# jonathan-laurent/AlphaZero.jl

Measured on AMD Instinct MI355X. Metric: self-play MCTS sims/sec (Connect-Four, 4096 parallel games per GPU), higher is better.
Workload: dtype f32

## Files before the change

### alphazero.jl_amd/csrc/azhip.hip

```cpp
#include "engine.h"

static thread_local std::string g_err;
int fail(int code, const char* fmt, ...) {
  char buf[512];
  va_list ap;
  va_start(ap, fmt);
  vsnprintf(buf, sizeof buf, fmt, ap);
  va_end(ap);
  g_err = buf;
  return code;
}
extern "C" const char* az_last_error(void) { return g_err.c_str(); }
extern "C" int az_abi_version(void) { return AZ_ABI_VERSION; }
extern "C" int az_abi_struct_size(int32_t which) {
  switch (which) {
    case AZ_STRUCT_ENGINE_CFG: return (int)sizeof(az_engine_cfg);
    case AZ_STRUCT_MOVE_REC: return (int)sizeof(az_move_rec);
    case AZ_STRUCT_GAME_REC: return (int)sizeof(az_game_rec);
    case AZ_STRUCT_TRACE_BUF: return (int)sizeof(az_trace_buf);
    case AZ_STRUCT_SELFPLAY_STATS: return (int)sizeof(az_selfplay_stats);
    case AZ_STRUCT_SAMPLE: return (int)sizeof(az_sample);
    case AZ_STRUCT_DATASET_INFO: return (int)sizeof(az_dataset_info);
    case AZ_STRUCT_LEARNING_STATUS: return (int)sizeof(az_learning_status_t);
    case AZ_STRUCT_TRAIN_CFG: return (int)sizeof(az_train_cfg);
// ... 349 lines not shown
    AZCHK(dalloc(e, &e->d_next, (size_t)2 * e->io_cap)); AZCHK(dalloc(e, &e->d_term, e->io_cap)); AZCHK(dalloc(e, &e->d_reward, e->io_cap));
    AZCHK(dalloc(e, &e->d_nodebuf, 512));
    AZCHK(dalloc(e, &e->d_visits, (size_t)e->io_cap * (AZ_MAX_ACTIONS + 1)));
    e->nn_cap = e->io_cap;
    AZCHK(dalloc(e, &e->d_hfeat, (size_t)e->nn_cap * gi.P * std::max(64, c->num_filters), false));
    AZCHK(dalloc(e, &e->d_X, (size_t)e->nn_cap * gi.C * gi.P)); AZCHK(dalloc(e, &e->d_A, (size_t)e->nn_cap * gi.A));
    AZCHK(dalloc(e, &e->d_P, (size_t)e->nn_cap * std::max(16, gi.APAD))); AZCHK(dalloc(e, &e->d_V, e->nn_cap)); AZCHK(dalloc(e, &e->d_Pinv, e->nn_cap));
    AZCHK(dalloc(e, &e->d_tmp_env, e->nn_cap)); AZCHK(dalloc(e, &e->d_iota, e->nn_cap)); AZCHK(dalloc(e, &e->d_ntmp, 1));
    HIPCHK(hipHostMalloc((void**)&e->h_env, sizeof(GEnv) * (size_t)e->nn_cap, hipHostMallocDefault));
    HIPCHK(hipHostMalloc((void**)&e->h_n, sizeof(int), hipHostMallocDefault));
    HIPCHK(hipHostMalloc((void**)&e->h_pv, sizeof(float) * (size_t)e->nn_cap * (gi.A + 1), hipHostMallocDefault));
    hipLaunchKernelGGL(k_iota, dim3((e->nn_cap + 255) / 256), dim3(256), 0, e->stream, e->d_iota, e->nn_cap);
    memset(&e->net, 0, sizeof e->net);
    memset(&e->net16, 0, sizeof e->net16);
    { const char* tw = getenv("AZHIP_TOWER"); e->tower_pick = tw ? atoi(tw) : 0; }
    { const char* mx = getenv("AZHIP_TOWER_MIXED"); e->tower_mixed = mx && atoi(mx) != 0; }
    { const char* hd = getenv("AZHIP_HEADS"); e->heads_pick = hd ? atoi(hd) : 0; }
    { const char* ep = getenv("AZHIP_XCH_EPOCH0"); e->xch_epoch = ep ? strtoull(ep, nullptr, 0) : 0; }
    { hipDeviceProp_t pr; HIPCHK(hipGetDeviceProperties(&pr, c->device)); e->num_cu = pr.multiProcessorCount; }
    AZCHK(net_set_kernel_attrs(e));
    { const char* ta = getenv("AZHIP_TREE_ATOMIC"); const int m = ta ? atoi(ta) : 0; v.bk_mode = m == 1 || m == 2 ? m : 0; }
    { const char* ts = getenv("AZHIP_TREE_SORT"); e->tree_sort = ts && atoi(ts) != 0 ? 1 : 0; }
    if (e->tree_sort) { AZCHK(dalloc(e, &e->d_perm, (size_t)2 * G)); AZCHK(dalloc(e, &e->d_perm_prev, (size_t)2 * G)); }
    int ng = c->batch_size > 0 ? G / c->batch_size : 1;
    if (ng < 1) ng = 1;
    if (ng > AZ_MAX_GROUPS) ng = AZ_MAX_GROUPS;
    while (ng > 1 && G % ng != 0) --ng;
    const int Gh = G / ng;
    const int blk_group = (Gh * gi.APAD + 255) / 256, blk_all = (G * gi.APAD + 255) / 256;
    e->stat_words = (size_t)4 * ((size_t)blk_group * ng + blk_all);
    AZCHK(dalloc(e, &v.stat, e->stat_words));
// ... 498 lines not shown
  }
  if (e->fr_on) {
    FRArgs fa;
    fa.st = e->d_fr; fa.done = e->d_done; fa.done_off = e->d_done_off;
    fa.recs = e->d_phase ? e->d_phase : e->d_stage; fa.recs_cap = e->d_phase ? (long long)e->phase_cap : (long long)e->v.G * e->v.max_moves;
    fa.done_cap = e->done_cap; fa.total_games = e->total_games; fa.first_game_id = (uint32_t)e->first_game_id; fa.group = g; fa.host_words = e->d_fr_words;
    static const int bg_prio = getenv("AZHIP_BG_PRIO") ? atoi(getenv("AZHIP_BG_PRIO")) : 0;
    hipStream_t s3 = side ? e->fr_s[2] : s2;
    if (side) { HIPCHK(hipStreamWaitEvent(s2, e->fr_ev[0], 0)); HIPCHK(hipStreamWaitEvent(s3, e->fr_ev[0], 0)); }
    { DView mv = v; mv.low_prio = bg_prio ? 0 : 1; LAUNCH_ON(e, s3, AZ_K_MOVE, G, (k_move_fr<Gm>), (G + 255) / 256, 256, 0, mv, e->p, fa); }
    if (e->fr_kbg > 0) {
      AZCHK(ec_next_launch(e, &e->gv[g]));
      DView bv = e->gv[g];
      bv.run_k = e->fr_kbg; bv.low_prio = bg_prio ? 0 : 1;
      if (side && e->bg_signal) { bv.bg_stop = e->d_bg_stop; bv.bg_seq = e->bg_seq; }
      LAUNCH_ON(e, s2, AZ_K_EXPAND, G, (k_tree<Gm>), gb, 256, 0, bv, e->p, 0, 1, par ^ 1);
    }
    if (side) {
      HIPCHK(hipEventRecord(e->fr_ev[1], s2)); HIPCHK(hipStreamWaitEvent(st, e->fr_ev[1], 0));
      HIPCHK(hipEventRecord(e->fr_ev[2], s3)); HIPCHK(hipStreamWaitEvent(st, e->fr_ev[2], 0));
    }
    else if (split && e->cfg.oracle == AZ_ORACLE_RESNET) HIPCHK(hipStreamWaitEvent(st, e->ev_net[g], 0));
  }
  return AZ_OK;
}
template <class Gm> static int recover_split(az_engine* e) {
  AZCHK(sync_all(e));
  *e->h_xflag = 0;
  int xerr[AZ_MAX_GROUPS + 1], skipped[2 * (AZ_MAX_GROUPS + 1)];
  HIPCHK(hipMemcpy(xerr, e->d_xerr, sizeof xerr, hipMemcpyDeviceToHost));
  HIPCHK(hipMemcpy(skipped, e->d_skipped, sizeof skipped, hipMemcpyDeviceToHost));
// ... 503 lines not shown
    fs.next_game = e->next_game;
    HIPCHK(hipMemsetAsync(e->v.finished, 0, sizeof(int) * G, e->stream));
    AZCHK(start_games<Gm>(e, aslots_refill, agids, nullptr, 1, 1));
    dirty = true;
  }
  if (!e->d_phase && (done > 0 || nrec > 0)) {
    fs.resv = 0; e->fr_prev_done = 0; e->fr_prev_recs = 0; dirty = true;
  }
  if (dirty) {
    HIPCHK(hipMemcpyAsync(e->d_fr, &fs, sizeof fs, hipMemcpyHostToDevice, e->stream));
    HIPCHK(hipStreamSynchronize(e->stream));
  }
  e->active_slots = 0;
  for (int g = 0; g < AZ_MAX_GROUPS; ++g) { e->group_active[g] = g < e->ngroups ? std::max(0, fs.active[g]) : 0; e->active_slots += e->group_active[g]; }
  e->h_fr_words[0] = e->fr_prev_done; e->h_fr_words[1] = e->active_slots;
  return vm_grow(e, e->fr_round_waves * e->fr_k + 2);
}
template <class Gm> static int fr_step(az_engine* e, int nwaves) {
  for (int w = 0; w < nwaves; ++w) {
    if (e->active_slots == 0) break;
    const int seen_done = ((volatile int*)e->h_fr_words)[0], seen_active = ((volatile int*)e->h_fr_words)[1];
    if (seen_active == 0 || (e->total_games > 0 && e->d_phase && seen_done + e->fr_given_up >= e->total_games)) break;
    AZCHK(wave<Gm>(e, e->ngroups, 0));
    if (++e->fr_since_round >= e->fr_round_waves) AZCHK(fr_round<Gm>(e));
  }
  return fr_round<Gm>(e);
}

extern "C" int az_selfplay_step(az_engine* e, int32_t nwaves) {
  ENGINE(e);
  if (!e->running) return fail(AZ_ERR_STATE, "az_selfplay_begin has not been called");
// ... 371 lines not shown
```

### alphazero.jl_amd/csrc/engine.h

```cpp
#pragma once
#include <hip/hip_runtime.h>

#include <algorithm>
#include <chrono>
#include <cmath>
#include <cstdarg>
#include <cstdio>
#include <cstring>
#include <new>
#include <string>
#include <map>
#include <mutex>
#include <vector>
#include <unordered_set>

#include "../../include/az_numerics.h"
#include "../../include/azhip.h"
#include "games.h"
#include "resnet.h"
#include "resnet16.h"
#include "resnet16b.h"
#include "tree.h"

int fail(int code, const char* fmt, ...);
// ... 27 lines not shown
  }
  return false;
}

enum TowerForm : int {
  TW_AUTO = 0,
  TW_SPLIT = 2,
  TW_NTS = 3,
  TW_NTM = 7,
  TW_11 = 16,
  TW_P19 = 19,
  TW_P21C = 20,
  TW_P21 = 21,
  TW_B22 = 22,
  TW_32 = 32,
  TW_MIXED = -1
};
struct ProfRec { hipEvent_t a = nullptr, b = nullptr; int cls = 0; };
struct az_engine {
  az_engine_cfg cfg;
  GameInfo gi;
  int device;
  hipStream_t stream;
  DView v;
  DParams p;
  int ngroups;
  DView gv[AZ_MAX_GROUPS];
  hipStream_t gs[AZ_MAX_GROUPS];
  hipStream_t gt[AZ_MAX_GROUPS];
  hipEvent_t ev_tree[AZ_MAX_GROUPS], ev_net[AZ_MAX_GROUPS];
  float* g_hfeat[AZ_MAX_GROUPS];
// ... 14 lines not shown
  int tree_sort; int* d_perm; long long* d_perm_prev;
  ECEnt* d_ec; uint32_t ec_mask; uint32_t ec_seq; int* d_ec_claim; float* d_Phit; float* d_Vhit;
  size_t stat_words; std::vector<long long> h_stat;
  std::vector<int32_t> aborted_ids;
  std::vector<void*> net_allocs;
  bool net_loaded;
  std::vector<float> blob;
  NetDev net;
  Net16bDev net16b;
  Net16Dev net16;
  uint16_t* d_geo[GEO_COUNT];
  long long tower_hist[4];
  char last_tower[96];
  int heads_pick;
  int tower_pick;
  bool tower_mixed;
  int num_cu;
  int nn_cap;
  float* d_hfeat; float* d_X; float* d_A; float* d_P; float* d_V; float* d_Pinv;
  GEnv* d_tmp_env; int* d_iota; int* d_ntmp;
  GEnv* h_env; int* h_n; float* h_pv;
  int* d_slots; uint32_t* d_gids; GEnv* d_roots; uint32_t* d_moves; double* d_eta; int* d_offsets;
  az_move_rec* d_stage; unsigned long long* d_keys; int* d_actions; unsigned long long* d_next; signed char* d_term; float* d_reward;
  char* d_nodebuf;
  int* d_visits;
  int io_cap;
  bool running;
  int total_games, next_game, first_game_id, games_done, wave_in_move, active_slots;
  std::map<int, hipGraphExec_t> wave_graphs; int use_graphs;
  bool pending[AZ_MAX_GROUPS];
  int wave_par[AZ_MAX_GROUPS];
// ... 133 lines not shown
```

### alphazero.jl_amd/csrc/net_c4.hip

```cpp
#include "net_impl.h"
AZ_NET_GAME_TU(ConnectFour, c4)


template <int F, int NT> static int tower_timeline(az_engine* e, int32_t n, unsigned long long* out, int64_t cap) {
  using T = T16<ConnectFour, F, NT>;
  const int nb = (n + T::TB - 1) / T::TB;
  if (cap < (int64_t)nb * 8) return fail(AZ_ERR_CAPACITY, "need %d words", nb * 8);
  unsigned long long* d = nullptr;
  AZCHK(dalloc(e, &d, (size_t)nb * 8));
  HIPCHK(hipMemsetAsync(d, 0, sizeof(unsigned long long) * nb * 8, e->stream));
  std::vector<GEnv> envs(n, ConnectFour::init());
  HIPCHK(hipMemcpyAsync(e->d_tmp_env, envs.data(), sizeof(GEnv) * n, hipMemcpyHostToDevice, e->stream));
  HIPCHK(hipMemcpyAsync(e->d_ntmp, &n, sizeof(int), hipMemcpyHostToDevice, e->stream));
  Net16Dev nd = e->net16;
  for (int rep = 0; rep < 2; ++rep) {
    nd.dbg = rep ? d : nullptr;
    hipLaunchKernelGGL((k_tower16<ConnectFour, F, false, NT>), dim3(nb), dim3(T::THREADS), T::BYTES, e->stream, nd, e->d_tmp_env, e->d_iota, e->d_ntmp, n, (const float*)nullptr, e->d_hfeat);
  }
  HIPCHK(hipMemcpyAsync(out, d, sizeof(unsigned long long) * nb * 8, hipMemcpyDeviceToHost, e->stream));
  HIPCHK(hipStreamSynchronize(e->stream));
  e->allocs.pop_back();
  (void)hipFree(d);
  return AZ_OK;
}
// ... 106 lines not shown
```

### alphazero.jl_amd/csrc/net_impl.h

```cpp
#pragma once
#include "engine.h"

template <class T> static constexpr double geo_frac() { return T::Geo::tab.cost / (9.0 * (T::RPAD / 16)); }
template <class T_, int ID_, bool OK_, int HIST_> struct FormFp32 {
  using T = T_;
  static constexpr int ID = ID_, HIST = HIST_;
  static constexpr bool OK = OK_, BF16 = false;
  static const Net16Dev& net(const az_engine* e) { return e->net16; }
  static constexpr double frac() { return geo_frac<T>(); }
};
template <class Gm, int F, int NT, int ID_, int HIST_> struct Form16 : FormFp32<T16<Gm, F, NT>, ID_, (NT > 0), HIST_> {
  template <bool FP> static constexpr auto K = &k_tower16<Gm, F, FP, NT>;
  static void name(char* s, size_t n, const char* g) { snprintf(s, n, "k_tower16<%s,%d,NT=%d>", g, F, NT); }
};
template <class Gm, int F> struct FormSplit : FormFp32<T16S<Gm, F>, TW_SPLIT, F == 128, 0> {
  template <bool FP> static constexpr auto K = &k_tower16s<Gm, F, FP>;
  static void name(char* s, size_t n, const char* g) { snprintf(s, n, "k_tower16s<%s,%d>", g, F); }
};
template <class Gm, int F, int NT0, int NT1, int ID_> struct FormPaired : FormFp32<T16P<Gm, F, NT0, NT1>, ID_, F == 64, 2> {
  template <bool FP> static constexpr auto K = &k_tower16x2<Gm, F, FP, NT0, NT1>;
  static void name(char* s, size_t n, const char* g) {
    if (NT0 == 11) snprintf(s, n, "k_tower16x2<%s,%d>", g, F);
    else snprintf(s, n, "k_tower16x2<%s,%d,NT=%d>", g, F, NT0 + NT1);
  }
};
template <class Gm, int F> struct FormPairedC : FormFp32<T16P<Gm, F>, TW_P21C, F == 64, 2> {
  template <bool FP> static constexpr auto K = &k_tower16x2c<Gm, F, FP>;
  static void name(char* s, size_t n, const char* g) { snprintf(s, n, "k_tower16x2c<%s,%d>", g, F); }
};
template <class Gm, int F> struct FormMixed : FormFp32<T16P<Gm, F>, TW_MIXED, F == 64, 2> {
  using T7 = T16P<Gm, F, 10, 9>;
  template <bool FP> static constexpr auto K = &k_tower16x2m<Gm, F, FP>;
  static void name(char* s, size_t n, const char* g) { snprintf(s, n, "k_tower16x2m<%s,%d>", g, F); }
};
template <class Gm, int F> struct Form32 {
  struct T { static constexpr int TB = TOWER_ROWS / Gm::P, THREADS = TowerCfg<F>::THREADS, BYTES = TowerLds<F>::BYTES; };
  static constexpr int ID = TW_32, HIST = 3;
  static constexpr bool OK = true, BF16 = false;
  template <bool FP> static constexpr auto K = &k_tower<Gm, F, FP>;
  static const NetDev& net(const az_engine* e) { return e->net; }
  static constexpr double frac() { return 1.0; }
  static void name(char* s, size_t n, const char* g) { snprintf(s, n, "k_tower<%s,%d>", g, F); }
};
template <class Gm, int F, int NT, int ID_, int HIST_> struct Form16b {
  using T = T16B<Gm, F, NT>;
  static constexpr int ID = ID_, HIST = HIST_;
  static constexpr bool OK = NT != 22 || F == 128, BF16 = true;
  template <bool FP> static constexpr auto K = &k_tower16b<Gm, F, FP, NT>;
  static const Net16bDev& net(const az_engine* e) { return e->net16b; }
// ... 2 lines not shown
};
template <class... D> struct FormList {};
template <class Gm, int F> using Forms = FormList<
    FormSplit<Gm, F>, Form16<Gm, F, NTS<Gm>, TW_NTS, 1>, Form16<Gm, F, NTM<Gm>, TW_NTM, 3>, Form16<Gm, F, 11, TW_11, 2>,
    FormPaired<Gm, F, 11, 10, TW_P21>, FormPaired<Gm, F, 10, 9, TW_P19>, FormPairedC<Gm, F>, Form32<Gm, F>,
    Form16b<Gm, F, NTS<Gm>, TW_NTS, 1>, Form16b<Gm, F, 11, TW_11, 2>, Form16b<Gm, F, 22, TW_B22, 3>>;

template <class D, bool FP> static int set_form_attr() {
  if constexpr (D::OK) HIPCHK(hipFuncSetAttribute(reinterpret_cast<const void*>(D::template K<FP>), hipFuncAttributeMaxDynamicSharedMemorySize, D::T::BYTES));
  return AZ_OK;
}
template <class Gm, int F, class... D> static int set_kernel_attrs_f(FormList<D...>) {
  int r = AZ_OK;
  (void)(((r = set_form_attr<D, false>()) == AZ_OK && (r = set_form_attr<D, true>()) == AZ_OK) && ...);
  AZCHK(r);
  AZCHK((set_form_attr<FormMixed<Gm, F>, false>()));
  HIPCHK(hipFuncSetAttribute(reinterpret_cast<const void*>(&k_heads16<Gm, F, true>), hipFuncAttributeMaxDynamicSharedMemorySize, H16<Gm, F, true>::BYTES));
  HIPCHK(hipFuncSetAttribute(reinterpret_cast<const void*>(&k_heads16<Gm, F, false>), hipFuncAttributeMaxDynamicSharedMemorySize, H16<Gm, F, false>::BYTES));
  return AZ_OK;
}
template <class T> static int upload_geo(az_engine* e) {
  using G = typename T::Geo;
  if (e->d_geo[T::GEO]) return AZ_OK;
  std::vector<uint16_t> h((size_t)10 * G::RPAD);
  for (int i = 0; i < G::RPAD; ++i) h[i] = G::tab.pos[i];
  for (int i = 0; i < 9 * G::RPAD; ++i) h[G::RPAD + i] = G::tab.nbr[i];
  uint16_t* d = nullptr;
  AZCHK(dalloc(e, &d, h.size(), false));
  HIPCHK(hipMemcpyAsync(d, h.data(), h.size() * sizeof(uint16_t), hipMemcpyHostToDevice, e->stream));
  HIPCHK(hipStreamSynchronize(e->stream));
  e->d_geo[T::GEO] = d;
// ... 89 lines not shown
template <class Gm, int F>
static int launch_heads(az_engine* e, hipStream_t st, const float* hfeat, const GEnv* envs, const int* eslots, const int* n_ptr, int n_max,
                        const float* Amask, float* Pout, float* Vout, float* Pinv, int pstride) {
  const bool small = e->heads_pick == 16 || (e->heads_pick != 32 && (n_max <= HEADS16_MAX_BOARDS || e->ngroups == 1));
  const int tiles = (n_max + 15) / 16;
  if (e->net.hd16_ok && small && 2 * tiles <= (e->num_cu > 0 ? e->num_cu : 256))
    LAUNCH_ON(e, st, AZ_K_HEADS, n_max, (k_heads16<Gm, F, true>), 2 * tiles, (H16<Gm, F, true>::THREADS), (H16<Gm, F, true>::BYTES), e->net, envs, eslots, n_ptr, n_max, Amask, hfeat, Pout, Vout, Pinv, pstride);
  else if (e->net.hd16_ok && small)
    LAUNCH_ON(e, st, AZ_K_HEADS, n_max, (k_heads16<Gm, F, false>), tiles, (H16<Gm, F, false>::THREADS), (H16<Gm, F, false>::BYTES), e->net, envs, eslots, n_ptr, n_max, Amask, hfeat, Pout, Vout, Pinv, pstride);
  else if (e->net.hd_ok)
    LAUNCH_ON(e, st, AZ_K_HEADS, n_max, (k_heads_mfma<Gm, F>), (n_max + 31) / 32, 64 * (F / 32 + HEADS_NPT<Gm>), 0, e->net, envs, eslots, n_ptr, n_max, Amask, hfeat, Pout, Vout, Pinv, pstride);
  else
    LAUNCH_ON(e, st, AZ_K_HEADS, n_max, (k_heads<Gm, F>), (n_max + 3) / 4, 4 * (F + HEADS_LP<Gm>), 0, e->net, envs, eslots, n_ptr, n_max, Amask, hfeat, Pout, Vout, Pinv, pstride);
  return AZ_OK;
}
struct TowerIn { float* hfeat; const GEnv* envs; const int* eslots; const int* n_ptr; const float* X; int* xerr; };
static const char* game_name(const az_engine* e) {
  static const char* const gn[] = {"ConnectFour", "TicTacToe", "Mancala", "Go9Planes"};
  return gn[e->cfg.game];
}
template <class D, bool FROM_PLANES> static int launch_form(az_engine* e, hipStream_t st, int n, const TowerIn& in) {
  if constexpr (!D::OK) return fail(AZ_ERR_STATE, "tower form %d does not exist for this network", (int)D::ID);
  else {
    using T = typename D::T;
    D::name(e->last_tower, sizeof e->last_tower, game_name(e));
    e->tower_hist[D::HIST]++;
    e->next_exec = D::frac();
    const int tiles = (n + T::TB - 1) / T::TB;
    if constexpr (D::ID == TW_SPLIT) {
      unsigned long long* xa; unsigned long long ep;
      AZCHK(xch_slot<typename T::Game>(e, in.hfeat, &xa, &ep));
      LAUNCH_ON(e, st, AZ_K_TOWER, n, (D::template K<FROM_PLANES>), T::SPLIT * tiles, T::THREADS, T::BYTES, D::net(e), in.envs, in.eslots, in.n_ptr, n, in.X, in.hfeat,
                xa, ep, in.xerr, e->d_xflag);
    } else
      LAUNCH_ON(e, st, AZ_K_TOWER, n, (D::template K<FROM_PLANES>), tiles, T::THREADS, T::BYTES, D::net(e), in.envs, in.eslots, in.n_ptr, n, in.X, in.hfeat);
    return AZ_OK;
  }
}
template <class Gm, int F, bool FROM_PLANES, class... D>
static int launch_tower(FormList<D...>, az_engine* e, hipStream_t st, int form, int n, const TowerIn& in) {
  const bool bf16 = e->cfg.net_bf16 != 0;
  int r = 1;
  (void)((D::ID == form && D::BF16 == bf16 && ((r = launch_form<D, FROM_PLANES>(e, st, n, in)), true)) || ...);
  return r <= 0 ? r : fail(AZ_ERR_STATE, "no tower form %d", form);
}
template <class Gm, int F, bool FROM_PLANES> static int launch_tower(az_engine* e, hipStream_t st, int form, int n, const TowerIn& in) {
  return launch_tower<Gm, F, FROM_PLANES>(Forms<Gm, F>{}, e, st, form, n, in);
}
template <class Gm, int F, bool FROM_PLANES>
static int launch_net_f(az_engine* e, hipStream_t st, float* hfeat, const GEnv* envs, const int* eslots, const int* n_ptr, int n_max, const float* X,
                        const float* Amask, float* Pout, float* Vout, float* Pinv, int pstride) {
  if (n_max <= 0) return AZ_OK;
  AZCHK((launch_tower<Gm, F, FROM_PLANES>(e, st, pick_tower<Gm, F>(e, n_max), n_max, TowerIn{hfeat, envs, eslots, n_ptr, X, e->v.err})));
  return launch_heads<Gm, F>(e, st, hfeat, envs, eslots, n_ptr, n_max, Amask, Pout, Vout, Pinv, pstride);
}
template <class Gm, bool FROM_PLANES>
static int launch_net(az_engine* e, hipStream_t st, float* hfeat, const GEnv* envs, const int* eslots, const int* n_ptr, int n_max, const float* X,
                      const float* Amask, float* Pout, float* Vout, float* Pinv, int pstride) {
  if (e->cfg.num_filters == 128) return launch_net_f<Gm, 128, FROM_PLANES>(e, st, hfeat, envs, eslots, n_ptr, n_max, X, Amask, Pout, Vout, Pinv, pstride);
  return launch_net_f<Gm, 64, FROM_PLANES>(e, st, hfeat, envs, eslots, n_ptr, n_max, X, Amask, Pout, Vout, Pinv, pstride);
}


template <class Gm, int F> static int wave_net_f(az_engine* e, int g, bool split, int nmax) {
  constexpr int L = Gm::APAD;
  const DView& v = e->gv[g];
  hipStream_t st = e->gs[g], sn = e->gt[g];
  const int G = v.G;
// ... 1 lines not shown
  const int N = std::max(1, std::min(G, nmax));
  const int* nev = v.n_eval + e->wave_par[g];
  const int* const eslots = v.eval_slots + (size_t)e->wave_par[g] * v.eval_stride;
  int npick = N;
  if (v.nleaf_host) { const int seen = ((volatile int*)e->h_nleaf)[g]; if (seen >= 0) npick = std::max(1, std::min(N, seen + seen / 8 + 8)); }
  int tw = pick_tower<Gm, F>(e, npick, N);
  if (tw == TW_P21 && e->fr_on && e->ngroups == 1 && e->tower_pick == 0 && e->fr_kbg > 0 && v.nleaf_host && v.needy_host) {
    const int cu = e->num_cu > 0 ? e->num_cu : 256;
    const int seen = ((volatile int*)e->h_nleaf)[g], needy = ((volatile int*)e->h_needy)[g];
    if (seen > 0) {
      constexpr int TB21 = T16P<Gm, 64>::TB;
      const int wgs = (seen + TB21 - 1) / TB21, rounds = (wgs + cu - 1) / cu, bg = (std::max(needy, 0) * L + 255) / 256;
      if (wgs > rounds * (cu - bg) - 14) tw = TW_P21C;
    }
  }
  const TowerIn in{e->g_hfeat[g], v.leaf_env, eslots, nev, nullptr, v.xerr};
  bool mixed = false;
  if constexpr (FormMixed<Gm, F>::OK) {
    using M = FormMixed<Gm, F>;
    using T8 = typename M::T; using T7 = typename M::T7;
    const int cu = e->num_cu > 0 ? e->num_cu : 256, first = cu * T8::TB;
    const int seen = v.nleaf_host ? ((volatile int*)e->h_nleaf)[g] : -1;
    if (tw == TW_P21 && e->tower_mixed && e->tower_pick == 0 && N > first && seen > first && seen + 16 <= first + cu * T7::TB) {
      mixed = true;
      M::name(e->last_tower, sizeof e->last_tower, game_name(e));
      e->tower_hist[M::HIST]++;
      e->next_exec = (first * geo_frac<T8>() + (seen - first) * geo_frac<T7>()) / (double)seen;
      LAUNCH_ON(e, sn, AZ_K_TOWER, N, (M::template K<false>), cu + (N - first + T7::TB - 1) / T7::TB, T8::THREADS, T8::BYTES, M::net(e), in.envs, in.eslots, in.n_ptr, N, in.X, in.hfeat, cu);
    }
  }
  if (!mixed) AZCHK((launch_tower<Gm, F, false>(e, sn, tw, N, in)));
  const bool fr = e->fr_on && split;
  if (e->bg_signal) {
    HIPCHK(hipEventRecord(e->fr_ev[3], sn));
    HIPCHK(hipStreamWaitEvent(e->fr_s[3], e->fr_ev[3], 0));
    hipLaunchKernelGGL(k_set_word, dim3(1), dim3(1), 0, e->fr_s[3], e->d_bg_stop, e->bg_seq);
  }
  if (split && !fr) { HIPCHK(hipEventRecord(e->ev_net[g], sn)); HIPCHK(hipStreamWaitEvent(st, e->ev_net[g], 0)); }
  AZCHK((launch_heads<Gm, F>(e, fr ? sn : st, e->g_hfeat[g], v.leaf_env, eslots, nev, N, (const float*)nullptr, v.Pout, v.Vout, (float*)nullptr, L)));
  if (fr) HIPCHK(hipEventRecord(e->ev_net[g], sn));
  return AZ_OK;
}
template <class Gm> static int wave_net(az_engine* e, int g, bool split, int nmax) {
  return e->cfg.num_filters == 128 ? wave_net_f<Gm, 128>(e, g, split, nmax) : wave_net_f<Gm, 64>(e, g, split, nmax);
}

// ... 16 lines not shown
```

### alphazero.jl_amd/csrc/resnet16.h

```cpp
#pragma once
#include <hip/hip_runtime.h>
#include <stdint.h>
#include "../../include/az_numerics.h"
#include "games.h"
#include "resnet.h"


enum GeoSlot {
  GEO_11,
  GEO_NTS,
  GEO_21,
  GEO_6,
  GEO_NTM,
  GEO_19,
  GEO_22,
  GEO_COUNT
};
struct Net16Dev {
  int nblocks;
  const float* stem_w;
  const float* stem_ss;
  const float4* conv_w;
  const float* conv_ss;
  const float4* head_w;
// ... 558 lines not shown

template <class T, bool FROM_PLANES>
__device__ __forceinline__ void tower16x2_body(const Net16Dev& net, const GEnv* __restrict__ leaf_env, const int* __restrict__ eval_slots, int n,
                                               const float* __restrict__ X, float* __restrict__ hfeat, int board0, const uint16_t* __restrict__ geo) {
  extern __shared__ __attribute__((aligned(16))) float lds[];
  float* buf = lds;
  float* planes = lds + T::BUF;
  uint16_t* nbr = (uint16_t*)(planes + T::PLANES);
  uint16_t* pos = nbr + 9 * T::RPAD;
  tower16_fill<T, FROM_PLANES>(buf, planes, nbr, pos, geo, leaf_env, eval_slots, X, n, board0, threadIdx.x);
  __syncthreads();
  const int wave = threadIdx.x >> 6, lane = threadIdx.x & 63;
  if (wave < T::CT) tower16_wave<T, FROM_PLANES, T::NT0, 0>(net, buf, planes, nbr, pos, wave, lane, n, board0, hfeat);
  else tower16_wave<T, FROM_PLANES, T::NT1, T::NT0>(net, buf, planes, nbr, pos, wave - T::CT, lane, n, board0, hfeat);
}
template <class Gm, int F, bool FROM_PLANES, int NT0 = 11, int NT1 = 10>
__global__ void __launch_bounds__(2 * T16Threads<F>::V, 1)
k_tower16x2(Net16Dev net, const GEnv* __restrict__ leaf_env, const int* __restrict__ eval_slots,
            const int* __restrict__ n_eval_ptr, int n_fixed, const float* __restrict__ X, float* __restrict__ hfeat) {
  using T = T16P<Gm, F, NT0, NT1>;
  const int n = FROM_PLANES ? n_fixed : *n_eval_ptr;
  const int board0 = blockIdx.x * T::TB;
  if (board0 >= n) return;
  tower16x2_body<T, FROM_PLANES>(net, leaf_env, eval_slots, n, X, hfeat, board0, net.geo[T::GEO]);
}
template <class Gm, int F, bool FROM_PLANES>
__global__ void __launch_bounds__(2 * T16Threads<F>::V, 1) __attribute__((amdgpu_num_vgpr(88)))
k_tower16x2c(Net16Dev net, const GEnv* __restrict__ leaf_env, const int* __restrict__ eval_slots,
             const int* __restrict__ n_eval_ptr, int n_fixed, const float* __restrict__ X, float* __restrict__ hfeat) {
  using T = T16P<Gm, F, 11, 10>;
  const int n = FROM_PLANES ? n_fixed : *n_eval_ptr;
  const int board0 = blockIdx.x * T::TB;
  if (board0 >= n) return;
  tower16x2_body<T, FROM_PLANES>(net, leaf_env, eval_slots, n, X, hfeat, board0, net.geo[T::GEO]);
}
template <class Gm, int F, bool FROM_PLANES>
__global__ void __launch_bounds__(2 * T16Threads<F>::V, 1)
k_tower16x2m(Net16Dev net, const GEnv* __restrict__ leaf_env, const int* __restrict__ eval_slots,
             const int* __restrict__ n_eval_ptr, int n_fixed, const float* __restrict__ X, float* __restrict__ hfeat, int first) {
  using T8 = T16P<Gm, F, 11, 10>;
  using T7 = T16P<Gm, F, 10, 9>;
  const int n = FROM_PLANES ? n_fixed : *n_eval_ptr;
  if ((int)blockIdx.x < first) {
    const int board0 = blockIdx.x * T8::TB;
    if (board0 >= n) return;
    tower16x2_body<T8, FROM_PLANES>(net, leaf_env, eval_slots, n, X, hfeat, board0, net.geo[T8::GEO]);
  } else {
    const int board0 = first * T8::TB + ((int)blockIdx.x - first) * T7::TB;
    if (board0 >= n) return;
    tower16x2_body<T7, FROM_PLANES>(net, leaf_env, eval_slots, n, X, hfeat, board0, net.geo[T7::GEO]);
  }
}

template <class Gm, int F> struct T16S : T16<Gm, F, NTS<Gm>> {
  static constexpr int SPLIT = 2, TPW = NTS<Gm>, CWL = F / 16 / SPLIT;
  static constexpr int WAVES = CWL, THREADS = 64 * WAVES;
  static constexpr int XCH_WORDS = 2 * TPW * 4 * THREADS;
};
template <class Gm, int F, bool FROM_PLANES>
__global__ void __launch_bounds__((T16S<Gm, F>::THREADS), 1)
k_tower16s(Net16Dev net, const GEnv* __restrict__ leaf_env, const int* __restrict__ eval_slots,
           const int* __restrict__ n_eval_ptr, int n_fixed, const float* __restrict__ X, float* __restrict__ hfeat,
           unsigned long long* __restrict__ xch, unsigned long long epoch, int* __restrict__ err, int* __restrict__ hflag) {
  using T = T16S<Gm, F>;
  extern __shared__ __attribute__((aligned(16))) float lds[];
  float* buf = lds;
  float* planes = lds + T::BUF;
  uint16_t* nbr = (uint16_t*)(planes + T::PLANES);
// ... 345 lines not shown
```

### alphazero.jl_amd/csrc/tree.h

```cpp
#pragma once
#include <hip/hip_runtime.h>
#include <stdint.h>
#include <type_traits>
#include "../../include/az_numerics.h"
#include "../../include/azhip.h"
#include "games.h"

enum { LEAF_NONE = 0, LEAF_NEW = 1, LEAF_TERMINAL = 2 };
enum { DERR_NODE_POOL = 1, DERR_HASH_FULL = 2, DERR_DEPTH = 3, DERR_MOVES = 4, DERR_NO_ROOT = 5 };

struct DParams {
  double gamma, cpuct, eps, alpha, prior_temp;
  int nsims, temp_len;
  int temp_xs[AZ_SCHED_MAX];
  double temp_ys[AZ_SCHED_MAX];
  uint64_t seed;
  int oracle, reset_every;
  double flip_p;
  int retire;
};

enum { SR_ACTIVE = 1, SR_MS_SHIFT = 8 };
struct alignas(64) SlotRec {
  unsigned long long root_a, root_b;
// ... 223 lines not shown
    double e = 0.0;
    if (a < Gm::A && ((m >> a) & 1)) e = eta[k++];
    v.eta[(size_t)slot * L + a] = e;
  }
}

template <class Gm> __device__ inline void set_link(char* nd, int act, uint32_t link) {
  using NL = NodeL<Gm>;
  ((uint16_t*)(nd + NL::OFF_LO))[act] = (uint16_t)(link & 0xffff);
  typename NL::hi_t* hp = (typename NL::hi_t*)(nd + NL::OFF_HI);
  *hp = (typename NL::hi_t)((*hp & ~((typename NL::hi_t)3 << (2 * act))) | ((typename NL::hi_t)(link >> 16) << (2 * act)));
}

struct KArgs { DView v; DParams p; };
template <class Gm>
__global__ void __launch_bounds__(256) __attribute__((amdgpu_num_vgpr(160))) k_tree(DView v_arg, DParams p_arg, int do_backup, int do_select, int par) {
  if (!v_arg.low_prio) __builtin_amdgcn_s_setprio(3);
  const DView& v = v_arg;
  constexpr int L = Gm::APAD;
  using NL = NodeL<Gm>;
  __shared__ int s_new[4], s_hit[4], s_evl[4], s_sims[4], s_trav[4], s_need[4], s_base, s_nbase;
  const int tid = blockIdx.x * blockDim.x + threadIdx.x;
  const int lgrp = tid / L, lane = tid % L;
  const int wl = threadIdx.x & 63, w = threadIdx.x >> 6, gbase = wl & ~(L - 1);
  int nlive = v.G;
  const int* map = v.perm;
  if (v.fr && !do_backup && v.bg_list) { nlive = v.bg_cnt[par ^ 1]; map = v.bg_list + (size_t)(par ^ 1) * v.eval_stride; }
  const bool live = lgrp < nlive;
  const int slot_in = live ? (map ? map[lgrp] : lgrp) : 0;
  const bool links_ok = v.cap_nodes <= LINK_MAX;
  unsigned long long* dbg = (v.dbg && blockIdx.x == 0 && threadIdx.x == 0) ? v.dbg : nullptr;
  if (dbg) dbg[0] = __builtin_readcyclecounter();
  if (__hip_atomic_load(v.xerr, __ATOMIC_RELAXED, __HIP_MEMORY_SCOPE_AGENT) == (int)DERR_EXCHANGE) {
    if (blockIdx.x == 0 && threadIdx.x == 0 && (do_backup || !v.fr)) atomicAdd(v.skipped + (do_select ? 0 : 1), 1);
    return;
  }

  const SlotRec s0 = v.sr[slot_in];
  unsigned long long st = (v.path + (size_t)slot_in * v.max_depth)[lane < v.max_depth ? lane : 0];
  GEnv lenv = v.leaf_env[slot_in];
  int kind = s0.leaf_kd & 3, depth = (s0.leaf_kd >> 2) & 0x0fffffff, e0 = s0.eidx, nc = s0.node_count;
  GEnv root0 = s0.root();
  uint32_t epoch0 = s0.epoch, ins = s0.leaf_ins;
  int ridx = s0.root_idx, active0 = s0.active;
  int claim0 = -1; uint32_t cmeta0 = 0;
  if (v.ec) { const int2 c2 = ((const int2*)v.ec_claim)[slot_in]; claim0 = c2.x; cmeta0 = (uint32_t)c2.y; }
#define AZ_PIN(x) asm volatile("" : "+v"(x))
  AZ_PIN(kind); AZ_PIN(depth); AZ_PIN(e0); AZ_PIN(nc); AZ_PIN(st); AZ_PIN(root0.a); AZ_PIN(root0.b); AZ_PIN(root0.fin);
// ... 283 lines not shown
  if (isnew) {
    int base = s_base;
    for (int i = 0; i < w; ++i) base += s_new[i];
    const int e = base + __popcll(bal & ((1ULL << wl) - 1ULL));
    sr->eidx = e;
    (v.eval_slots + (size_t)par * v.eval_stride)[e] = slot;
  }
  if (needy && v.fr) {
    int base = s_nbase;
    for (int i = 0; i < w; ++i) base += s_need[i];
    (v.bg_list + (size_t)par * v.eval_stride)[base + __popcll(baln & ((1ULL << wl) - 1ULL))] = slot;
  }
  if (v.ec && head && kind == LEAF_NEW) ((int2*)v.ec_claim)[slot] = make_int2(ishit ? -1 : claim, ishit ? 0 : (int)cmeta);
  if (dbg) dbg[6] = __builtin_readcyclecounter();
}

template <class Gm>
__host__ __device__ inline float rollout_value(GEnv g, uint64_t seed, uint32_t game_id, uint32_t move, uint32_t sim) {
  const bool wp = Gm::white_playing(g);
  az_rng r = az_rng_make(seed, game_id, move, AZ_RNG_ROLLOUT);
  r.ctr[3] = sim * 1024u;
  double wr = 0.0;
  for (int ply = 0; ply < 1024 && !(g.fin & 1); ++ply) {
    const uint32_t m = Gm::mask(g);
    int acts[AZ_MAX_ACTIONS], n = 0;
    for (int a = 0; a < Gm::A; ++a) if ((m >> a) & 1) acts[n++] = a;
    int k = (int)(az_rng_f64(&r) * (double)n);
    if (k >= n) k = n - 1;
    Gm::play(g, acts[k]);
    wr = (double)Gm::white_reward(g);
// ... 383 lines not shown
```

Before: 8.843 million.

## Add low-VGPR background tree kernel and adaptive paired tower split

Introduces k_tree_bg, a copy of the tree kernel capped at 56 VGPRs, for background expansion so it can co-reside with the tower kernel. In the background path, one thread reads the exchange-error flag into shared memory instead of every thread reading it. It also replaces the separate mixed tower kernel with an adaptive paired split inside k_tower16x2 that balances heavy and light tiles across CU slots, on by default when the free-running single-group mode is active. The VM growth bound is widened to account for background launches. The 56-VGPR cap may cause register spills, and the extra split logic adds per-block overhead.

Measured after the change: 8.792 million. About the same (-0.6%).

```diff
diff --git a/alphazero.jl_amd/csrc/azhip.hip b/alphazero.jl_amd/csrc/azhip.hip
--- a/alphazero.jl_amd/csrc/azhip.hip
+++ b/alphazero.jl_amd/csrc/azhip.hip
@@ -387,7 +387,7 @@
     memset(&e->net, 0, sizeof e->net);
     memset(&e->net16, 0, sizeof e->net16);
     { const char* tw = getenv("AZHIP_TOWER"); e->tower_pick = tw ? atoi(tw) : 0; }
-    { const char* mx = getenv("AZHIP_TOWER_MIXED"); e->tower_mixed = mx && atoi(mx) != 0; }
+    { const char* mx = getenv("AZHIP_TOWER_MIXED"); e->tower_mixed = mx ? (atoi(mx) != 0 ? 1 : 0) : -1; }
     { const char* hd = getenv("AZHIP_HEADS"); e->heads_pick = hd ? atoi(hd) : 0; }
     { const char* ep = getenv("AZHIP_XCH_EPOCH0"); e->xch_epoch = ep ? strtoull(ep, nullptr, 0) : 0; }
     { hipDeviceProp_t pr; HIPCHK(hipGetDeviceProperties(&pr, c->device)); e->num_cu = pr.multiProcessorCount; }
@@ -916,7 +916,7 @@
       DView bv = e->gv[g];
       bv.run_k = e->fr_kbg; bv.low_prio = bg_prio ? 0 : 1;
       if (side && e->bg_signal) { bv.bg_stop = e->d_bg_stop; bv.bg_seq = e->bg_seq; }
-      LAUNCH_ON(e, s2, AZ_K_EXPAND, G, (k_tree<Gm>), gb, 256, 0, bv, e->p, 0, 1, par ^ 1);
+      LAUNCH_ON(e, s2, AZ_K_EXPAND, G, (k_tree_bg<Gm>), gb, 256, 0, bv, e->p, 0, 1, par ^ 1);
     }
     if (side) {
       HIPCHK(hipEventRecord(e->fr_ev[1], s2)); HIPCHK(hipStreamWaitEvent(st, e->fr_ev[1], 0));
@@ -1450,7 +1450,7 @@
   e->active_slots = 0;
   for (int g = 0; g < AZ_MAX_GROUPS; ++g) { e->group_active[g] = g < e->ngroups ? std::max(0, fs.active[g]) : 0; e->active_slots += e->group_active[g]; }
   e->h_fr_words[0] = e->fr_prev_done; e->h_fr_words[1] = e->active_slots;
-  return vm_grow(e, e->fr_round_waves * e->fr_k + 2);
+  return vm_grow(e, (int)std::min<long long>((long long)e->fr_round_waves * (e->fr_k + 1 + e->fr_kbg) + 2, 1 << 30));
 }
 template <class Gm> static int fr_step(az_engine* e, int nwaves) {
   for (int w = 0; w < nwaves; ++w) {
diff --git a/alphazero.jl_amd/csrc/engine.h b/alphazero.jl_amd/csrc/engine.h
--- a/alphazero.jl_amd/csrc/engine.h
+++ b/alphazero.jl_amd/csrc/engine.h
@@ -65,7 +65,6 @@
   TW_P21 = 21,
   TW_B22 = 22,
   TW_32 = 32,
-  TW_MIXED = -1
 };
 struct ProfRec { hipEvent_t a = nullptr, b = nullptr; int cls = 0; };
 struct az_engine {
@@ -110,7 +109,7 @@
   char last_tower[96];
   int heads_pick;
   int tower_pick;
-  bool tower_mixed;
+  int tower_mixed;
   int num_cu;
   int nn_cap;
   float* d_hfeat; float* d_X; float* d_A; float* d_P; float* d_V; float* d_Pinv;
diff --git a/alphazero.jl_amd/csrc/net_c4.hip b/alphazero.jl_amd/csrc/net_c4.hip
--- a/alphazero.jl_amd/csrc/net_c4.hip
+++ b/alphazero.jl_amd/csrc/net_c4.hip
@@ -2,6 +2,16 @@
 AZ_NET_GAME_TU(ConnectFour, c4)
 
 
+extern "C" int az_debug_paired_split(int32_t n, int32_t places, int32_t margin, int32_t* heavy, int32_t* wgs, double* frac, int32_t* board0, int64_t cap) {
+  if (!heavy || !wgs || !frac || n < 1 || places < 1 || margin < 0) return fail(AZ_ERR_BAD_ARG, "bad argument");
+  using T8 = T16P<ConnectFour, 64>;
+  using T7 = T16P<ConnectFour, 64, 10, 9>;
+  const PairedSplit sp = paired_split(n, places, margin, T8::TB, T7::TB);
+  *heavy = sp.heavy; *wgs = sp.wgs;
+  *frac = paired_exec_frac(sp, n, T8::TB, geo_frac<T8>(), geo_frac<T7>());
+  for (int i = 0; board0 && i < sp.wgs && i < cap; ++i) board0[i] = paired_board0(sp, i, T8::TB, T7::TB);
+  return AZ_OK;
+}
 template <int F, int NT> static int tower_timeline(az_engine* e, int32_t n, unsigned long long* out, int64_t cap) {
   using T = T16<ConnectFour, F, NT>;
   const int nb = (n + T::TB - 1) / T::TB;
diff --git a/alphazero.jl_amd/csrc/net_impl.h b/alphazero.jl_amd/csrc/net_impl.h
--- a/alphazero.jl_amd/csrc/net_impl.h
+++ b/alphazero.jl_amd/csrc/net_impl.h
@@ -28,11 +28,7 @@
   template <bool FP> static constexpr auto K = &k_tower16x2c<Gm, F, FP>;
   static void name(char* s, size_t n, const char* g) { snprintf(s, n, "k_tower16x2c<%s,%d>", g, F); }
 };
-template <class Gm, int F> struct FormMixed : FormFp32<T16P<Gm, F>, TW_MIXED, F == 64, 2> {
-  using T7 = T16P<Gm, F, 10, 9>;
-  template <bool FP> static constexpr auto K = &k_tower16x2m<Gm, F, FP>;
-  static void name(char* s, size_t n, const char* g) { snprintf(s, n, "k_tower16x2m<%s,%d>", g, F); }
-};
+template <class Gm, int F> static constexpr bool PAIRED_ADAPTIVE = F == 64 && std::is_same<Gm, ConnectFour>::value;
 template <class Gm, int F> struct Form32 {
   struct T { static constexpr int TB = TOWER_ROWS / Gm::P, THREADS = TowerCfg<F>::THREADS, BYTES = TowerLds<F>::BYTES; };
   static constexpr int ID = TW_32, HIST = 3;
@@ -65,7 +61,6 @@
   int r = AZ_OK;
   (void)(((r = set_form_attr<D, false>()) == AZ_OK && (r = set_form_attr<D, true>()) == AZ_OK) && ...);
   AZCHK(r);
-  AZCHK((set_form_attr<FormMixed<Gm, F>, false>()));
   HIPCHK(hipFuncSetAttribute(reinterpret_cast<const void*>(&k_heads16<Gm, F, true>), hipFuncAttributeMaxDynamicSharedMemorySize, H16<Gm, F, true>::BYTES));
   HIPCHK(hipFuncSetAttribute(reinterpret_cast<const void*>(&k_heads16<Gm, F, false>), hipFuncAttributeMaxDynamicSharedMemorySize, H16<Gm, F, false>::BYTES));
   return AZ_OK;
@@ -185,7 +180,7 @@
     LAUNCH_ON(e, st, AZ_K_HEADS, n_max, (k_heads<Gm, F>), (n_max + 3) / 4, 4 * (F + HEADS_LP<Gm>), 0, e->net, envs, eslots, n_ptr, n_max, Amask, hfeat, Pout, Vout, Pinv, pstride);
   return AZ_OK;
 }
-struct TowerIn { float* hfeat; const GEnv* envs; const int* eslots; const int* n_ptr; const float* X; int* xerr; };
+struct TowerIn { float* hfeat; const GEnv* envs; const int* eslots; const int* n_ptr; const float* X; int* xerr; int slots = 0; int expect = 0; bool forced = false; };
 static const char* game_name(const az_engine* e) {
   static const char* const gn[] = {"ConnectFour", "TicTacToe", "Mancala", "Go9Planes"};
   return gn[e->cfg.game];
@@ -203,6 +198,19 @@
       AZCHK(xch_slot<typename T::Game>(e, in.hfeat, &xa, &ep));
       LAUNCH_ON(e, st, AZ_K_TOWER, n, (D::template K<FROM_PLANES>), T::SPLIT * tiles, T::THREADS, T::BYTES, D::net(e), in.envs, in.eslots, in.n_ptr, n, in.X, in.hfeat,
                 xa, ep, in.xerr, e->d_xflag);
+    } else if constexpr (D::ID == TW_P21 || D::ID == TW_P19) {
+      int grid = tiles, slots = 0;
+      if constexpr (D::ID == TW_P21 && PAIRED_ADAPTIVE<typename T::Game, T::FILT>) {
+        if (in.slots > 0) {
+          using T7 = T16P<typename T::Game, T::FILT, 10, 9>;
+          slots = in.slots;
+          grid = paired_split(n, slots, PAIRED_MARGIN, T::TB, T7::TB).wgs;
+          const int ne = in.expect > 0 ? std::min(in.expect, n) : n;
+          e->next_exec = paired_exec_frac(paired_split(ne, slots, PAIRED_MARGIN, T::TB, T7::TB), ne, T::TB, geo_frac<T>(), geo_frac<T7>());
+          if (in.forced) snprintf(e->last_tower, sizeof e->last_tower, "k_tower16x2m<%s,%d>", game_name(e), (int)T::FILT);
+        }
+      }
+      LAUNCH_ON(e, st, AZ_K_TOWER, n, (D::template K<FROM_PLANES>), grid, T::THREADS, T::BYTES, D::net(e), in.envs, in.eslots, in.n_ptr, n, in.X, in.hfeat, slots);
     } else
       LAUNCH_ON(e, st, AZ_K_TOWER, n, (D::template K<FROM_PLANES>), tiles, T::THREADS, T::BYTES, D::net(e), in.envs, in.eslots, in.n_ptr, n, in.X, in.hfeat);
     return AZ_OK;
@@ -222,7 +230,10 @@
 static int launch_net_f(az_engine* e, hipStream_t st, float* hfeat, const GEnv* envs, const int* eslots, const int* n_ptr, int n_max, const float* X,
                         const float* Amask, float* Pout, float* Vout, float* Pinv, int pstride) {
   if (n_max <= 0) return AZ_OK;
-  AZCHK((launch_tower<Gm, F, FROM_PLANES>(e, st, pick_tower<Gm, F>(e, n_max), n_max, TowerIn{hfeat, envs, eslots, n_ptr, X, e->v.err})));
+  TowerIn in{hfeat, envs, eslots, n_ptr, X, e->v.err};
+  const int tw = pick_tower<Gm, F>(e, n_max);
+  if (tw == TW_P21 && e->tower_pick == 0 && e->tower_mixed != 0) { in.slots = e->num_cu > 0 ? e->num_cu : 256; in.forced = e->tower_mixed > 0; }
+  AZCHK((launch_tower<Gm, F, FROM_PLANES>(e, st, tw, n_max, in)));
   return launch_heads<Gm, F>(e, st, hfeat, envs, eslots, n_ptr, n_max, Amask, Pout, Vout, Pinv, pstride);
 }
 template <class Gm, bool FROM_PLANES>
@@ -254,22 +265,13 @@
       if (wgs > rounds * (cu - bg) - 14) tw = TW_P21C;
     }
   }
-  const TowerIn in{e->g_hfeat[g], v.leaf_env, eslots, nev, nullptr, v.xerr};
-  bool mixed = false;
-  if constexpr (FormMixed<Gm, F>::OK) {
-    using M = FormMixed<Gm, F>;
-    using T8 = typename M::T; using T7 = typename M::T7;
-    const int cu = e->num_cu > 0 ? e->num_cu : 256, first = cu * T8::TB;
-    const int seen = v.nleaf_host ? ((volatile int*)e->h_nleaf)[g] : -1;
-    if (tw == TW_P21 && e->tower_mixed && e->tower_pick == 0 && N > first && seen > first && seen + 16 <= first + cu * T7::TB) {
-      mixed = true;
-      M::name(e->last_tower, sizeof e->last_tower, game_name(e));
-      e->tower_hist[M::HIST]++;
-      e->next_exec = (first * geo_frac<T8>() + (seen - first) * geo_frac<T7>()) / (double)seen;
-      LAUNCH_ON(e, sn, AZ_K_TOWER, N, (M::template K<false>), cu + (N - first + T7::TB - 1) / T7::TB, T8::THREADS, T8::BYTES, M::net(e), in.envs, in.eslots, in.n_ptr, N, in.X, in.hfeat, cu);
-    }
-  }
-  if (!mixed) AZCHK((launch_tower<Gm, F, false>(e, sn, tw, N, in)));
+  TowerIn in{e->g_hfeat[g], v.leaf_env, eslots, nev, nullptr, v.xerr};
+  if (tw == TW_P21 && e->tower_pick == 0 && (e->tower_mixed > 0 || (e->tower_mixed < 0 && e->fr_on && e->ngroups == 1))) {
+    in.slots = e->num_cu > 0 ? e->num_cu : 256;
+    in.expect = v.nleaf_host ? ((volatile int*)e->h_nleaf)[g] : 0;
+    in.forced = e->tower_mixed > 0;
+  }
+  AZCHK((launch_tower<Gm, F, false>(e, sn, tw, N, in)));
   const bool fr = e->fr_on && split;
   if (e->bg_signal) {
     HIPCHK(hipEventRecord(e->fr_ev[3], sn));
diff --git a/alphazero.jl_amd/csrc/resnet16.h b/alphazero.jl_amd/csrc/resnet16.h
--- a/alphazero.jl_amd/csrc/resnet16.h
+++ b/alphazero.jl_amd/csrc/resnet16.h
@@ -596,12 +596,42 @@
   if (wave < T::CT) tower16_wave<T, FROM_PLANES, T::NT0, 0>(net, buf, planes, nbr, pos, wave, lane, n, board0, hfeat);
   else tower16_wave<T, FROM_PLANES, T::NT1, T::NT0>(net, buf, planes, nbr, pos, wave - T::CT, lane, n, board0, hfeat);
 }
+static constexpr int PAIRED_MARGIN = 0;
+struct PairedSplit { int heavy, wgs; };
+__host__ __device__ inline PairedSplit paired_split(int n, int places, int margin, int tb8, int tb7) {
+  const int R = (n + tb8 * places - 1) / (tb8 * places), S = R * places - margin, d = tb8 - tb7;
+  if (n <= 0) return PairedSplit{0, 0};
+  if (S <= 0) { const int h = (n + tb8 - 1) / tb8; return PairedSplit{h, h}; }
+  int heavy = n > tb7 * S ? (n - tb7 * S + d - 1) / d : 0;
+  if (heavy > S) heavy = S;
+  const int rest = n - tb8 * heavy;
+  return PairedSplit{heavy, heavy + (rest > 0 ? (rest + tb7 - 1) / tb7 : 0)};
+}
+__host__ __device__ inline int paired_board0(const PairedSplit& sp, int wg, int tb8, int tb7) {
+  return wg < sp.heavy ? wg * tb8 : sp.heavy * tb8 + (wg - sp.heavy) * tb7;
+}
+inline double paired_exec_frac(const PairedSplit& sp, int n, int tb8, double f8, double f7) {
+  const int n8 = sp.heavy * tb8 < n ? sp.heavy * tb8 : n;
+  return n > 0 ? (n8 * f8 + (n - n8) * f7) / (double)n : f8;
+}
 template <class Gm, int F, bool FROM_PLANES, int NT0 = 11, int NT1 = 10>
 __global__ void __launch_bounds__(2 * T16Threads<F>::V, 1)
 k_tower16x2(Net16Dev net, const GEnv* __restrict__ leaf_env, const int* __restrict__ eval_slots,
-            const int* __restrict__ n_eval_ptr, int n_fixed, const float* __restrict__ X, float* __restrict__ hfeat) {
+            const int* __restrict__ n_eval_ptr, int n_fixed, const float* __restrict__ X, float* __restrict__ hfeat, int slots) {
   using T = T16P<Gm, F, NT0, NT1>;
   const int n = FROM_PLANES ? n_fixed : *n_eval_ptr;
+  if constexpr (NT0 == 11 && NT1 == 10) {
+    if (slots > 0) {
+      using T7 = T16P<Gm, F, 10, 9>;
+      const PairedSplit sp = paired_split(n, slots, PAIRED_MARGIN, T::TB, T7::TB);
+      if ((int)blockIdx.x >= sp.heavy) {
+        const int board0 = paired_board0(sp, blockIdx.x, T::TB, T7::TB);
+        if (board0 >= n) return;
+        tower16x2_body<T7, FROM_PLANES>(net, leaf_env, eval_slots, n, X, hfeat, board0, net.geo[T7::GEO]);
+        return;
+      }
+    }
+  }
   const int board0 = blockIdx.x * T::TB;
   if (board0 >= n) return;
   tower16x2_body<T, FROM_PLANES>(net, leaf_env, eval_slots, n, X, hfeat, board0, net.geo[T::GEO]);
@@ -616,24 +646,6 @@
   if (board0 >= n) return;
   tower16x2_body<T, FROM_PLANES>(net, leaf_env, eval_slots, n, X, hfeat, board0, net.geo[T::GEO]);
 }
-template <class Gm, int F, bool FROM_PLANES>
-__global__ void __launch_bounds__(2 * T16Threads<F>::V, 1)
-k_tower16x2m(Net16Dev net, const GEnv* __restrict__ leaf_env, const int* __restrict__ eval_slots,
-             const int* __restrict__ n_eval_ptr, int n_fixed, const float* __restrict__ X, float* __restrict__ hfeat, int first) {
-  using T8 = T16P<Gm, F, 11, 10>;
-  using T7 = T16P<Gm, F, 10, 9>;
-  const int n = FROM_PLANES ? n_fixed : *n_eval_ptr;
-  if ((int)blockIdx.x < first) {
-    const int board0 = blockIdx.x * T8::TB;
-    if (board0 >= n) return;
-    tower16x2_body<T8, FROM_PLANES>(net, leaf_env, eval_slots, n, X, hfeat, board0, net.geo[T8::GEO]);
-  } else {
-    const int board0 = first * T8::TB + ((int)blockIdx.x - first) * T7::TB;
-    if (board0 >= n) return;
-    tower16x2_body<T7, FROM_PLANES>(net, leaf_env, eval_slots, n, X, hfeat, board0, net.geo[T7::GEO]);
-  }
-}
-
 template <class Gm, int F> struct T16S : T16<Gm, F, NTS<Gm>> {
   static constexpr int SPLIT = 2, TPW = NTS<Gm>, CWL = F / 16 / SPLIT;
   static constexpr int WAVES = CWL, THREADS = 64 * WAVES;
diff --git a/alphazero.jl_amd/csrc/tree.h b/alphazero.jl_amd/csrc/tree.h
--- a/alphazero.jl_amd/csrc/tree.h
+++ b/alphazero.jl_amd/csrc/tree.h
@@ -261,7 +261,7 @@
 
 struct KArgs { DView v; DParams p; };
 template <class Gm>
-__global__ void __launch_bounds__(256) __attribute__((amdgpu_num_vgpr(160))) k_tree(DView v_arg, DParams p_arg, int do_backup, int do_select, int par) {
+__device__ __forceinline__ void tree_body(const DView& v_arg, const DParams& p_arg, int do_backup, int do_select, int par) {
   if (!v_arg.low_prio) __builtin_amdgcn_s_setprio(3);
   const DView& v = v_arg;
   constexpr int L = Gm::APAD;
@@ -278,7 +278,14 @@
   const bool links_ok = v.cap_nodes <= LINK_MAX;
   unsigned long long* dbg = (v.dbg && blockIdx.x == 0 && threadIdx.x == 0) ? v.dbg : nullptr;
   if (dbg) dbg[0] = __builtin_readcyclecounter();
-  if (__hip_atomic_load(v.xerr, __ATOMIC_RELAXED, __HIP_MEMORY_SCOPE_AGENT) == (int)DERR_EXCHANGE) {
+  int xe;
+  if (v.fr && !do_backup) {
+    __shared__ int s_xerr;
+    if (threadIdx.x == 0) s_xerr = __hip_atomic_load(v.xerr, __ATOMIC_RELAXED, __HIP_MEMORY_SCOPE_AGENT);
+    __syncthreads();
+    xe = s_xerr;
+  } else xe = __hip_atomic_load(v.xerr, __ATOMIC_RELAXED, __HIP_MEMORY_SCOPE_AGENT);
+  if (xe == (int)DERR_EXCHANGE) {
     if (blockIdx.x == 0 && threadIdx.x == 0 && (do_backup || !v.fr)) atomicAdd(v.skipped + (do_select ? 0 : 1), 1);
     return;
   }
@@ -592,6 +599,14 @@
   if (v.ec && head && kind == LEAF_NEW) ((int2*)v.ec_claim)[slot] = make_int2(ishit ? -1 : claim, ishit ? 0 : (int)cmeta);
   if (dbg) dbg[6] = __builtin_readcyclecounter();
 }
+template <class Gm>
+__global__ void __launch_bounds__(256) __attribute__((amdgpu_num_vgpr(160))) k_tree(DView v_arg, DParams p_arg, int do_backup, int do_select, int par) {
+  tree_body<Gm>(v_arg, p_arg, do_backup, do_select, par);
+}
+template <class Gm>
+__global__ void __launch_bounds__(256) __attribute__((amdgpu_num_vgpr(56))) k_tree_bg(DView v_arg, DParams p_arg, int do_backup, int do_select, int par) {
+  tree_body<Gm>(v_arg, p_arg, do_backup, do_select, par);
+}
 
 template <class Gm>
 __host__ __device__ inline float rollout_value(GEnv g, uint64_t seed, uint32_t game_id, uint32_t move, uint32_t sim) {
```
